# TuringLang/NormalizingFlows.jl

Measured on AMD Instinct MI355X. Metric: elbo_samples_per_sec, higher is better.
Workload: dtype f32; 1 GPU; reverse-KL ELBO step: RealNVP d=64, 8 affine couplings, conditioner 32-64-64-32 (hdims [64,64]), diag-Gaussian target, Philox base draws, Adam; batch_per_gpu=65536, global_batch=65536, params=133632, parallelism=dp1 (sample-sharded, one all-reduce of P+1 floats per step), nf_comm_size=1, lib_comm_hung=False, step_form=nf_elbo_step (whole iteration inside the library), init=Glorot-uniform weights, zero biases (Flux default), weight_cache=nf_ctx_set_weight_cache(ctx, 1), as train_flow's loop sets it

## Files before the change

normalizingflows.jl_amd/csrc/nf_api.hip:

```cpp
#include <cmath>
#include <cstdlib>

#include "nf_common.h"

int nf_launch_base_sample(nf_ctx *, int, int, long, uint64_t, uint64_t, uint32_t, void *, void *);
int nf_launch_base_logpdf(nf_ctx *, int, int, long, const void *, void *);
int nf_launch_base_unwhiten(nf_ctx *, int dtype, int kind, int d, long N, const void *mu, const void *scale, void *x);
int nf_launch_base_general_logpdf(nf_ctx *, int dtype, int kind, int d, long N, const void *mu, const void *scale, double logdet,
                                  const void *x, void *logq_out, void *corr_out, void *zbuf);
int nf_launch_base_general_score(nf_ctx *, int dtype, int kind, int d, long N, const void *mu, const void *scale, double logdet,
                                 const void *x, void *logq_out, void *score_out, double gscale, void *zbuf);
long nf_target_nblocks(long N);
int nf_launch_target(nf_ctx *, int, const nf_target *, int, long, const void *, const void *, const void *, void *,
                     void *, double, void *, double *, double, int joint_d);
long nf_sum2_nblocks(long N);
int nf_launch_sum2(nf_ctx *, int, long, const void *, const void *, void *, double *, double);
int nf_launch_finish_sum(nf_ctx *, const double *, long, int, double *, float *, double *, unsigned *bump = nullptr);
int nf_launch_reduce_slabs(nf_ctx *, int, const void *, int, long, void *);
long nf_adam_nblocks(long P);
int nf_launch_adam(nf_ctx *, int, void *, const void *, void *, void *, long, double, double, double, double, long,
                   double *);
int nf_launch_sgd(nf_ctx *, int, void *, const void *, void *, long, double, double, double *);
int nf_launch_fill(nf_ctx *, int, void *, long, double);
int nf_launch_base_sample_tiled(nf_ctx *, int d, long N, uint64_t seed, uint64_t off, uint32_t stream, float *xt, float *logq);
// ... 12 lines not shown
long nf_affine_chain_grid(nf_ctx *, long N);
int nf_affine_chain_elbo(nf_ctx *, const nf_flow_desc *, long N, uint64_t seed, uint64_t off, uint32_t stream,
                         const nf_target *target, float *yt, float *gt, double gscale, double *partial,
                         double pscale, float *stash = nullptr, const uint32_t *stream_ptr = nullptr);
long nf_affine_epilogue_blocks(const nf_flow_desc *desc);
bool nf_affine_chain_fkl_ok(const nf_flow_desc *desc);
int nf_affine_chain_fkl(nf_ctx *, const nf_flow_desc *, const float *ys, long N, float *gt, double gscale, double *partial,
                        double pscale, float *stash);
int nf_affine_epilogue(nf_ctx *, const nf_flow_desc *, int mode, const float *slab, int nslab, float *g, const double *lpart,
                       int nlpart, float *theta, float *m, float *v, double lr, double b1, double b2, double eps, unsigned t_val,
                       unsigned *t_ptr, double *gpart);
size_t nf_affine_stash_floats(const nf_flow_desc *desc, long N);
bool nf_affine_stash_pays(const nf_flow_desc *desc);
bool nf_affine_fused_ok(const nf_flow_desc *desc);
int nf_affine_bwd_stashed(nf_ctx *, const nf_flow_desc *, float *stash, float *ybar, const float *lbar, float lbar_const, long N,
                          float *slab, long slab_stride, int grid, bool inv_dir = false);
long nf_affine_slab_floats(const nf_flow_desc *desc);
int nf_affine_reduce_slabs(nf_ctx *, const nf_flow_desc *, const float *slab, int nslab, float *g,
                           const double *lpart = nullptr, int nlpart = 0, float *lout = nullptr);
int nf_affine_bwd(nf_ctx *, const nf_flow_desc *, int k, const float *theta, float *y, float *ybar, const float *lbar,
                  float lbar_const, long N, float *slab, long slab_stride, int grid);
int nf_affine_bwd_all(nf_ctx *, const nf_flow_desc *, float *y, float *ybar, const float *lbar, float lbar_const, long N,
                      float *slab, long slab_stride, int grid, bool inv_dir = false);

bool nf_wide_supported(const nf_flow_desc *desc);
int nf_wide_pack(nf_ctx *, const nf_flow_desc *, const float *theta);
int nf_wide_apply(nf_ctx *, const nf_flow_desc *, int k, bool inverse, float *xt, long N, float *ladj, int accumulate);
size_t nf_wide_bwd_ws_floats(nf_ctx *, const nf_flow_desc *, long N);
int nf_wide_bwd(nf_ctx *, const nf_flow_desc *, float *state, float *gbar, const float *lbar, float lbar_const, long N,
                float *ws, float *g_out, bool inv_dir = false);
size_t nf_wide_train_ws_floats(nf_ctx *, const nf_flow_desc *, long N);
// ... 1068 lines not shown

  if (tiled) {
    float *zt = (float *)z, *gt = (float *)gbar;
    NF_TRY(nf_launch_layout_convert(ctx, desc->d, N, (const float *)ys, zt, 1));
    if (stash) {
      NF_TRY(coupling_pack(ctx, desc, (const float *)theta));
      const long stride = coupling_slab_floats(ctx, desc, N);
      long nslab = 0, npart = 0;
      for (long o = 0; o < N; o += stash_nc) {
        const long nc = N - o < stash_nc ? N - o : stash_nc;
        const int gc = coupling_bwd_grid(ctx, desc, nc);
        NF_TRY(nf_affine_chain(ctx, desc, true, zt + o * desc->d, nc, (float *)ladj + o, stash));
        NF_TRY(nf_launch_target_tiled(ctx, &q0, desc->d, nc, zt + o * desc->d, nullptr, (const float *)ladj + o, gt + o * desc->d, -inv,
                                      nullptr, partial + npart, -inv));
        NF_TRY(nf_affine_bwd_stashed(ctx, desc, stash, gt + o * desc->d, nullptr, (float)(-inv), nc, (float *)slab + nslab * stride,
                                     stride, gc, true));
        nslab += gc;
        npart += nf_target_tiled_nblocks(nc);
      }
      NF_TRY(nf_launch_finish_sum(ctx, partial, npart, 0, nullptr, (float *)out + P, nullptr));
      return nf_affine_reduce_slabs(ctx, desc, (const float *)slab, (int)nslab, (float *)out);
    }
    NF_TRY(coupling_chain_tiled(ctx, desc, true, (const float *)theta, zt, N, (float *)ladj, -1, rqs_tape));
    NF_TRY(nf_launch_target_tiled(ctx, &q0, desc->d, N, zt, nullptr, (const float *)ladj, gt, -inv, nullptr, partial, -inv));
    NF_TRY(nf_launch_finish_sum(ctx, partial, nb, 0, nullptr, (float *)out + P, nullptr));
    return coupling_inv_bwd(ctx, desc, (const float *)theta, zt, gt, (float)(-inv), N, (float *)slab, grid, (float *)out, rqs_tape);
  }
  if (hf) {
    NF_TRY(nf_hf_apply(ctx, desc, 0, nf_layer_count(desc), true, theta, ys, N, z, ladj));
    NF_TRY(nf_launch_target(ctx, dt, &q0, desc->d, N, z, nullptr, ladj, nullptr, gbar, -inv, nullptr, partial, -inv, 0));
    NF_TRY(nf_hf_bwd_inv(ctx, desc, theta, ys, gbar, -inv, N, out, fws));
// ... 458 lines not shown
  (void)result;
  char *slab = cv.take<char>(slabf * es);
  char *sws = cv.take<char>(simple_ws);
  float *stash = stash_b ? cv.take<float>(stash_b / 4) : nullptr;
  void *rqs_tape = rqs_b ? (void *)cv.take<char>(rqs_b) : nullptr;

  if (fusable) {
    float *xt = (float *)x, *gt = (float *)gbar;
    NF_TRY(coupling_pack(ctx, desc, (const float *)theta));
    if (stash) {
      const long stride = coupling_slab_floats(ctx, desc, N);
      long nslab = 0, npart = 0;
      for (long o = 0; o < N; o += stash_nc) {
        const long nc = N - o < stash_nc ? N - o : stash_nc;
        const int gc = coupling_bwd_grid(ctx, desc, nc);
        NF_TRY(fused_chain_elbo(ctx, desc, target, nc, seed, sample_offset + (uint64_t)o, stream_id, xt + o * desc->d,
                                gt + o * desc->d, -inv, partial + npart, -inv, stash));
        NF_TRY(nf_affine_bwd_stashed(ctx, desc, stash, gt + o * desc->d, nullptr, (float)(-inv), nc,
                                     (float *)slab + nslab * stride, stride, gc));
        nslab += gc;
        npart += nf_affine_chain_grid(ctx, nc);
      }
      return nf_affine_reduce_slabs(ctx, desc, (const float *)slab, (int)nslab, (float *)out, partial, (int)npart, (float *)out + P);
    }
    NF_TRY(fused_chain_elbo(ctx, desc, target, N, seed, sample_offset, stream_id, xt, gt, -inv, partial, -inv,
                            is_nsf(desc) ? (float *)rqs_tape : nullptr));
    if (is_nsf(desc)) {
      NF_TRY(nf_launch_finish_sum(ctx, partial, fused_chain_grid(ctx, desc, N), 0, nullptr, (float *)out + P, nullptr));
      return realnvp_bwd(ctx, desc, (const float *)theta, xt, gt, nullptr, (float)(-inv), N, (float *)slab, grid, (float *)out,
                         nullptr, 0, nullptr, rqs_tape);
    }
    return realnvp_bwd(ctx, desc, (const float *)theta, xt, gt, nullptr, (float)(-inv), N, (float *)slab, grid, (float *)out,
                       partial, (int)nf_affine_chain_grid(ctx, N), (float *)out + P);
  }
// ... 19 lines not shown
      NF_TRY(nf_launch_base_logpdf_tiled(ctx, desc->d, N, xt, (float *)logq));
    } else {
      NF_TRY(nf_launch_base_sample_tiled(ctx, desc->d, N, seed, sample_offset, stream_id, xt, (float *)logq));
    }
    if (stash) {
      NF_TRY(coupling_pack(ctx, desc, (const float *)theta));
      const long stride = coupling_slab_floats(ctx, desc, N);
      long nslab = 0, npart = 0;
      for (long o = 0; o < N; o += stash_nc) {
        const long nc = N - o < stash_nc ? N - o : stash_nc;
        const int gc = coupling_bwd_grid(ctx, desc, nc);
        NF_TRY(nf_affine_chain(ctx, desc, false, xt + o * desc->d, nc, (float *)ladj + o, stash));
        NF_TRY(nf_launch_target_tiled(ctx, target, desc->d, nc, xt + o * desc->d, (const float *)logq + o, (const float *)ladj + o,
                                      gt + o * desc->d, -inv, nullptr, partial + npart, -inv));
        NF_TRY(nf_affine_bwd_stashed(ctx, desc, stash, gt + o * desc->d, nullptr, (float)(-inv), nc,
                                     (float *)slab + nslab * stride, stride, gc));
        nslab += gc;
        npart += nf_target_tiled_nblocks(nc);
      }
      NF_TRY(nf_launch_finish_sum(ctx, partial, npart, 0, nullptr, (float *)out + P, nullptr));
      return nf_affine_reduce_slabs(ctx, desc, (const float *)slab, (int)nslab, (float *)out);
    }
    NF_TRY(coupling_chain_tiled(ctx, desc, false, (const float *)theta, xt, N, (float *)ladj, -1, rqs_tape));
    NF_TRY(nf_launch_target_tiled(ctx, target, desc->d, N, xt, (const float *)logq, (const float *)ladj, gt, -inv,
                                  nullptr, partial, -inv));
    NF_TRY(nf_launch_finish_sum(ctx, partial, nb, 0, nullptr, (float *)out + P, nullptr));
    NF_TRY(realnvp_bwd(ctx, desc, (const float *)theta, xt, gt, nullptr, (float)(-inv), N, (float *)slab, grid,
                       (float *)out, nullptr, 0, nullptr, rqs_tape));
  } else {
    if (simple_step) {
      NF_TRY(nf_target_check(target, desc->d));
// ... 83 lines not shown
  for (int i = 0; i < d->n_hidden && i < 4; ++i) mix((unsigned long long)d->hdims[i]);
  return h | (1ull << 63);
}
static bool step_fusable(nf_ctx *ctx, const nf_flow_desc *desc, const nf_target *target, long N) {
  constexpr bool off = false;
  if (off || flow_base(desc) || is_composite(desc) || desc->dtype != NF_DTYPE_F32) return false;
  if (!(desc->kind == NF_KIND_REALNVP && nf_affine_supported(desc))) return false;
  if (!elbo_fusable(desc, target, nullptr)) return false;
  return affine_stash_chunk(ctx, desc, N) > 0;
}
static size_t step_fused_need(nf_ctx *ctx, const nf_flow_desc *desc, long N) {
  const size_t te = tiled_elems(desc, N);
  const long nb = nf_target_tiled_nblocks(N);
  const long nb_alloc = nb < ctx->num_cu ? ctx->num_cu : nb;
  const long snc = affine_stash_chunk(ctx, desc, N);
  return 2 * carve_bytes(te * 4) + carve_bytes((size_t)nb_alloc * 8) +
         carve_bytes(chunked_slab_floats(ctx, desc, N, snc, coupling_slab_floats(ctx, desc, N)) * 4) +
         carve_bytes(snc ? affine_stash_bytes(ctx, desc, snc) : 0) + carve_bytes((size_t)nf_affine_epilogue_blocks(desc) * 8);
}
static int elbo_step_fused(nf_ctx *ctx, const nf_flow_desc *desc, const nf_target *target, float *theta, float *m, float *v,
                           long N, uint64_t seed, uint32_t step_val, uint32_t *step_ptr, double lr, double beta1, double beta2,
                           double eps) {
  const long P = nf_param_count(desc);
  const int world = ctx->comm ? ctx->comm_size : 1;
  const long Ng = N * world;
  const uint64_t off0 = (uint64_t)(ctx->comm ? ctx->comm_rank : 0) * (uint64_t)N;
  const double inv = 1.0 / (double)Ng;
  const size_t te = tiled_elems(desc, N);
  const long nb = nf_target_tiled_nblocks(N);
  const long nb_alloc = nb < ctx->num_cu ? ctx->num_cu : nb;
  const long stash_nc = affine_stash_chunk(ctx, desc, N);
  const long stride = coupling_slab_floats(ctx, desc, N);
  const size_t slabf = chunked_slab_floats(ctx, desc, N, stash_nc, stride);
  const size_t stash_b = affine_stash_bytes(ctx, desc, stash_nc);
  const long eblocks = nf_affine_epilogue_blocks(desc);
  NF_TRY(nf_ws_reserve(ctx, step_fused_need(ctx, desc, N)));
  Carver cv(ctx->ws);
  float *xt = cv.take<float>(te);
  float *gt = cv.take<float>(te);
  double *partial = cv.take<double>(nb_alloc);
  float *slab = cv.take<float>(slabf);
  float *stash = cv.take<float>(stash_b / 4);
  double *gpart = cv.take<double>(eblocks);
  float *gbuf = (float *)ctx->gbuf;
  constexpr bool repack = false;
  if (repack || !ctx->wimg_cache ||
      !(ctx->wimg && ctx->wimg_owner == (const void *)theta && ctx->wimg_sig == flow_sig(desc))) {
    NF_TRY(coupling_pack(ctx, desc, theta));
  }
  long nslab = 0, npart = 0;
  for (long o = 0; o < N; o += stash_nc) {
    const long nc = N - o < stash_nc ? N - o : stash_nc;
    const int gc = coupling_bwd_grid(ctx, desc, nc);
    NF_TRY(nf_affine_chain_elbo(ctx, desc, nc, seed, off0 + (uint64_t)o, step_val, target,
                                xt + o * desc->d, gt + o * desc->d, -inv, partial + npart, -inv, stash, step_ptr));
    NF_TRY(nf_affine_bwd_stashed(ctx, desc, stash, gt + o * desc->d, nullptr, (float)(-inv), nc, slab + nslab * stride, stride, gc));
    nslab += gc;
    npart += nf_affine_chain_grid(ctx, nc);
  }
  if (world == 1) {
    NF_TRY(nf_affine_epilogue(ctx, desc, 3, slab, (int)nslab, gbuf, partial, (int)npart, theta, m, v, lr, beta1, beta2, eps, step_val,
                              step_ptr, gpart));
  } else {
    NF_TRY(nf_affine_epilogue(ctx, desc, 1, slab, (int)nslab, gbuf, partial, (int)npart, nullptr, nullptr, nullptr, lr, beta1, beta2,
                              eps, step_val, nullptr, gpart));
    NF_TRY(nf_allreduce_grad_loss(ctx, NF_DTYPE_F32, gbuf, P + 1));
    NF_TRY(nf_affine_epilogue(ctx, desc, 2, nullptr, 0, gbuf, nullptr, 0, theta, m, v, lr, beta1, beta2, eps, step_val, step_ptr,
                              gpart));
  }
  NF_TRY(nf_launch_finish_sum(ctx, gpart, eblocks, 1, nullptr, gbuf + P + 1, nullptr, step_ptr));
  ctx->wimg_owner = theta;
// ... 230 lines not shown
  NF_TRY(nf_ws_reserve(ctx, fkl_step_need(ctx, desc, N)));
  Carver cv(ctx->ws);
  float *gt = cv.take<float>(tiled_elems(desc, N));
  double *partial = cv.take<double>(fkl_step_npart(ctx, N, stash_nc));
  float *slab = cv.take<float>(chunked_slab_floats(ctx, desc, N, stash_nc, stride));
  float *stash = cv.take<float>(affine_stash_bytes(ctx, desc, stash_nc) / 4);
  double *gpart = cv.take<double>(eblocks);
  float *gbuf = (float *)ctx->gbuf;
  if (!ctx->wimg_cache || !(ctx->wimg && ctx->wimg_owner == (const void *)theta && ctx->wimg_sig == flow_sig(desc)))
    NF_TRY(coupling_pack(ctx, desc, theta));
  long nslab = 0, npart = 0;
  for (long o = 0; o < N; o += stash_nc) {
    const long nc = N - o < stash_nc ? N - o : stash_nc;
    const int gc = coupling_bwd_grid(ctx, desc, nc);
    NF_TRY(nf_affine_chain_fkl(ctx, desc, ys + o * desc->d, nc, gt + o * desc->d, -inv, partial + npart, -inv, stash));
    NF_TRY(nf_affine_bwd_stashed(ctx, desc, stash, gt + o * desc->d, nullptr, (float)(-inv), nc, slab + nslab * stride, stride, gc, true));
    nslab += gc;
    npart += nf_affine_chain_grid(ctx, nc);
  }
  if (world == 1) {
    NF_TRY(nf_affine_epilogue(ctx, desc, 3, slab, (int)nslab, gbuf, partial, (int)npart, theta, m, v, lr, beta1, beta2, eps, step_val,
                              step_ptr, gpart));
  } else {
    NF_TRY(nf_affine_epilogue(ctx, desc, 1, slab, (int)nslab, gbuf, partial, (int)npart, nullptr, nullptr, nullptr, lr, beta1, beta2,
                              eps, step_val, nullptr, gpart));
    NF_TRY(nf_allreduce_grad_loss(ctx, NF_DTYPE_F32, gbuf, P + 1));
    NF_TRY(nf_affine_epilogue(ctx, desc, 2, nullptr, 0, gbuf, nullptr, 0, theta, m, v, lr, beta1, beta2, eps, step_val, step_ptr,
                              gpart));
  }
  NF_TRY(nf_launch_finish_sum(ctx, gpart, eblocks, 1, nullptr, gbuf + P + 1, nullptr, step_ptr));
  ctx->wimg_owner = theta;
// ... 225 lines not shown
```

normalizingflows.jl_amd/csrc/nf_coupling.hip:

```cpp
#include <cmath>
#include <cstdlib>

#include "nf_common.h"
#ifdef NF_COUPLING_SPLIT_SCALAR
#define NF_SPLIT_SCALAR
#endif
#ifdef NF_COUPLING_SLOPE_SCALAR
#define NF_SLOPE_SCALAR
#endif
#include "nf_mfma.h"
#include "nf_pack.h"
#include "nf_philox.h"
#include "nf_target_epilogue.h"

int nf_target_check(const nf_target *t, int d);

struct CouplingArgs {
  const float *theta;
  const float *img_s, *img_t;
  long long *trace;
  NetDims s, t;
  int d, c, m, par_t;
  long N;
};
// ... 532 lines not shown
          NF_CH_STAMP(tr, 4);
          buf ^= 1;
          continue;
        } else if (INVERSE ? (half == 1) : (half == 0)) {
          (void)x1_is_O;
          ls = coupling_step<G, INVERSE>(img_s, img_t, O, E, l31, hi);
        } else {
          ls = coupling_step<G, INVERSE>(img_s, img_t, E, O, l31, hi);
        }
        lsum += ls;
        __syncthreads();
        buf ^= 1;
      }
    }
    if (live) {
      if constexpr (!FKL) {
#pragma unroll
        for (int b = 0; b < G::CB; ++b)
#pragma unroll
          for (int r = 0; r < 16; ++r) {
            tile_store(io, tile_soff(b, r, 0), E[b][r]);
            tile_store(io, tile_soff(b, r, 1), O[b][r]);
          }
      }
      lsum += __shfl_xor(lsum, 32);
      if (!FUSED) {
        if (hi == 0 && valid) ladj[j] = INVERSE ? -lsum : lsum;
      }
    }
    if constexpr (FKL) {
      const TileIO gio = make_tile_io(fa.gt, tl, a.d, l31, hi);
// ... 491 lines not shown

template <class G, bool FULL>
__global__ __launch_bounds__(256, 1) void k_affine_bwd(CouplingArgs a, float *__restrict__ y, float *__restrict__ ybar,
                                                       const float *__restrict__ lbar, float lbar_const,
                                                       float *__restrict__ slab, long slab_stride) {
  extern __shared__ __attribute__((aligned(16))) float lds[];
  bwd_coupling<G, FULL>(a, y, ybar, lbar, lbar_const, slab, slab_stride, lds);
}

struct BwdAllArgs {
  const float *wimg;
  const unsigned char *wimg_b6t;
  long long *trace;
  int d, ncoup;
  long N;
};
template <class G, bool FULL, bool INVD>
__global__ __launch_bounds__(256, 1) void k_affine_bwd_all(BwdAllArgs aa, float *__restrict__ y, float *__restrict__ ybar,
                                                           const float *__restrict__ lbar, float lbar_const,
                                                           float *__restrict__ slab, long slab_stride) {
  extern __shared__ __attribute__((aligned(16))) float lds[];
#pragma unroll 1
  for (int step = 0; step < aa.ncoup; ++step) {
    const int k = INVD ? aa.ncoup - 1 - step : step;
    CouplingArgs a;
    a.theta = nullptr;
    a.img_s = aa.wimg + (size_t)(2 * k) * G::SIZE;
    a.img_t = a.img_s + G::SIZE;
    a.trace = k == 0 ? aa.trace : nullptr;
    a.d = aa.d;
// ... 417 lines not shown
#define NF_PAIR_BUF D6_BUF
#define NF_PAIR_PUT(NB, buf, s) split_to_lds<NB>(buf, s, l31, hi)
#define NF_PAIR_DW(IB, OB, as, buf, w, b) dw_accumulate_t6<IB, OB>(as, buf, w, b, l31, hi)
#endif
template <class G, bool PB6 = false, bool DW6 = false>
struct BwdPairLds {
  static_assert(!DW6 || (PB6 && G::CB <= 2 && G::H1B <= 2 && G::H2B <= 2), "triple buffers hold two blocks");
  static constexpr int D3 = 0, D2 = D3 + G::CB * 32 * NF_TS, D1 = D2 + G::H2B * 32 * NF_TS;
  static constexpr int PAIR = DW6 ? 2 * NF_PAIR_BUF / 4 : D1 + G::H1B * 32 * NF_TS;
  static constexpr int PAIRS = 4;
  static constexpr int IMG = PB6 ? B6TGeo<G>::BYTES / 4 : G::SIZE;
  static constexpr int FLOATS = (IMG + PAIRS * PAIR) > PAIRS * G::SIZE ? (IMG + PAIRS * PAIR) : PAIRS * G::SIZE;
  static constexpr size_t BYTES = (size_t)FLOATS * sizeof(float);
};

template <class G, bool PHASE_S, bool FULL, bool INVD, bool SLIM, bool PB6 = false, bool DW6 = false>
__device__ __forceinline__ void pair_produce(const CouplingArgs &a, const float *__restrict__ img, float *__restrict__ sp,
                                             StashFirst<G> &f, float *stash, int k, int ncoup, float *__restrict__ ybar,
                                             const float *__restrict__ lbar, float lbar_const, long tile, long next_tile,
                                             bool live, int l31, int hi, int par, long long *tr = nullptr) {
  using SG = StashGeo<G, SLIM>;
  using L = BwdPairLds<G, PB6, DW6>;
  char *bufa = reinterpret_cast<char *>(sp) + par * NF_PAIR_BUF, *bufb = reinterpret_cast<char *>(sp) + (par ^ 1) * NF_PAIR_BUF;
  if (!live) {
    __syncthreads();
    __syncthreads();
    __syncthreads();
    return;
  }
  NF_TS_STAMP(0);
  const long j = tile * NF_TILE + l31;
  const bool valid = FULL ? true : j < a.N;
  const int par_c = 1 - a.par_t;
  const TileIO gio = make_tile_io(ybar, tile, a.d, l31, hi);
  const StashIO st = make_stash_io(stash, tile * ncoup + k, SG::SIZE, true, l31, hi);
  constexpr int nbase = SG::NET0 + (PHASE_S ? 0 : SG::NETSZ);
  f32x16 g1[G::CB];
#pragma unroll
  for (int b = 0; b < G::CB; ++b)
#pragma unroll
    for (int r = 0; r < 16; ++r) g1[b][r] = tile_load(gio, tile_soff(b, r, a.par_t));
  const u32x4 mk = __builtin_amdgcn_raw_buffer_load_b128(st.rs, (hi * 32 + l31) * 16, (nbase + SG::MSK) * 4, 0);
  f32x16 gold[G::MB];
#pragma unroll
  for (int b = 0; b < G::MB; ++b)
#pragma unroll
    for (int r = 0; r < 16; ++r) gold[b][r] = tile_load(gio, tile_soff(b, r, par_c));
  const float lb = valid ? (lbar ? lbar[FULL ? j : (j < a.N ? j : 0)] : lbar_const) : 0.f;
  f32x16 d3[G::CB];
#pragma unroll
  for (int b = 0; b < G::CB; ++b)
#pragma unroll
    for (int r = 0; r < 16; ++r) {
      const bool ok = (b * 32 + nf_row(r, hi) < a.c) && valid;
      const float gv = g1[b][r];
      if (!PHASE_S) {
        d3[b][r] = ok ? (INVD ? -gv : gv) : 0.f;
      } else if (INVD) {
        const float sv = f.sv[b][r];
        tile_store(gio, tile_soff(b, r, a.par_t), nf_fdiv(gv, nf_exp(sv)));
        d3[b][r] = ok ? -(gv * f.uv[b][r] + lb) * (1.f - sv * sv) : 0.f;
      } else {
        const float sv = f.sv[b][r];
        tile_store(gio, tile_soff(b, r, a.par_t), gv * nf_exp(sv));
        d3[b][r] = ok ? (gv * f.uv[b][r] + lb) * (1.f - sv * sv) : 0.f;
      }
    }
  SplitC<DW6 ? G::CB : 1> s3;
  if constexpr (DW6) {
    split_C<G::CB>(d3, s3);
    NF_PAIR_PUT(G::CB, bufa, s3);
  } else {
    tile_to_scratch<G::CB>(sp + L::D3, d3, l31, hi);
  }
  unsigned m1[G::H1B], m2[G::H2B];
#pragma unroll
  for (int b = 0; b < G::H1B; ++b) m1[b] = mk[b];
#pragma unroll
  for (int b = 0; b < G::H2B; ++b) m2[b] = mk[2 + b];
  NF_TS_STAMP(1);
  __syncthreads();
  NF_TS_STAMP(2);
// ... 51 lines not shown
  if constexpr (DW6) dense_bwd_x_b6s<G::H1B, G::H2B>(wt + B6TGeo<G>::T2, s2, d1, l31, hi);
  else if constexpr (PB6) dense_bwd_x_b6<G::H1B, G::H2B>(wt + B6TGeo<G>::T2, d2, d1, l31, hi);
  else dense_bwd_x<G::H1B, G::H2B>(img + G::W2, d2, d1, l31, hi);
  apply_lrelu_grad<G::H1B>(d1, m1);
  if constexpr (DW6) {
    split_C<G::H1B>(d1, s1);
    NF_PAIR_PUT(G::H1B, bufa, s1);
  } else {
    tile_to_scratch<G::H1B>(sp + L::D1, d1, l31, hi);
  }
  }
  NF_TS_STAMP(5);
  __syncthreads();
  NF_TS_STAMP(6);
  if (PHASE_S && next_tile >= 0) stash_issue_first<G, SLIM>(f, stash, k, ncoup, next_tile, l31, hi);
  f32x16 g2[G::MB];
  if constexpr (DW6) dense_bwd_x_b6s<G::MB, G::H1B>(wt + B6TGeo<G>::T1, s1, g2, l31, hi);
  else if constexpr (PB6) dense_bwd_x_b6<G::MB, G::H1B>(wt + B6TGeo<G>::T1, d1, g2, l31, hi);
  else dense_bwd_x<G::MB, G::H1B>(img + G::W1, d1, g2, l31, hi);
#pragma unroll
  for (int b = 0; b < G::MB; ++b)
#pragma unroll
    for (int r = 0; r < 16; ++r) tile_store(gio, tile_soff(b, r, par_c), gold[b][r] + g2[b][r]);
  NF_TS_STAMP(7);
}

template <int NA, int NB>
__device__ __forceinline__ void consumer_split_and_request(const StashIO &st, int base, int voff, const float (&at)[NA][16], SplitT<NA> &s,
                                                           float (&bt)[NB][16]) {
  constexpr int NS = 2 * NA, NL = 4 * NB;
#pragma unroll
  for (int i = 0; i < NS; ++i) {
    const int ib = i >> 1, g = i & 1;
    float v[8];
#pragma unroll
    for (int j = 0; j < 8; ++j) v[j] = at[ib][8 * g + j];
#pragma unroll
    for (int l = i * NL / NS; l < (i + 1) * NL / NS; ++l) {
// ... 250 lines not shown
    if constexpr (PB6)
      stage_packed<BT::BYTES / 4, 512>(img, reinterpret_cast<const float *>(aa.wimg_b6t + (size_t)(2 * k + (is_s ? 0 : 1)) * BT::BYTES), tid);
    else
      stage_packed<G::SIZE, 512>(img, aa.wimg + (size_t)(2 * k + (is_s ? 0 : 1)) * G::SIZE, tid);
  };
  const long ntiles = (aa.N + NF_TILE - 1) / NF_TILE;
  const long tile0 = (long)blockIdx.x * 4 + pair, tstride = (long)gridDim.x * 4;
  const long wg0 = (long)blockIdx.x * 4;
  const int rounds = wg0 < ntiles ? (int)((ntiles - wg0 + tstride - 1) / tstride) : 0;
  if (role == 0) {
    StashFirst<G> f;
    if (INVD && tile0 < ntiles) stash_issue_first<G, SLIM>(f, stash, aa.ncoup - 1, aa.ncoup, tile0, l31, hi);
#pragma unroll 1
    for (int step = 0; step < aa.ncoup; ++step) {
      const int k = INVD ? aa.ncoup - 1 - step : step;
      CouplingArgs a;
      a.theta = nullptr;
      a.img_s = aa.wimg + (size_t)(2 * k) * G::SIZE;
      a.img_t = a.img_s + G::SIZE;
      a.trace = nullptr;
      a.d = aa.d;
      a.par_t = k & 1;
      a.c = (k & 1) ? aa.d / 2 : (aa.d + 1) / 2;
      a.m = aa.d - a.c;
      a.N = aa.N;
#pragma unroll 1
      for (int phase = 0; phase < 2; ++phase) {
        const bool is_s = INVD ? phase == 0 : phase == 1;
#ifdef NF_KERNEL_TRACE
        long long *trb = (aa.trace && blockIdx.x == 0 && tid == 64 * NF_TRACE_PAIR && step == 0) ? aa.trace + 32 + phase * 8 : nullptr;
#endif
        NF_TSB(0);
        stage_image(k, is_s);
        NF_TSB(1);
        __syncthreads();
        NF_TSB(2);
#pragma unroll 1
        for (int it = 0; it < rounds; ++it) {
          const long tile = tile0 + (long)it * tstride;
          const long nt = tile + tstride < ntiles ? tile + tstride : -1;
#ifdef NF_KERNEL_TRACE
          long long *tr = (aa.trace && blockIdx.x == 0 && tid == 64 * NF_TRACE_PAIR && step == 0 && it < 2) ? aa.trace + phase * 16 + it * 8 : nullptr;
#else
          long long *tr = nullptr;
#endif
          if (!is_s) pair_produce<G, false, FULL, INVD, SLIM, PB6, DW6>(a, img, sp, f, stash, k, aa.ncoup, ybar, lbar, lbar_const, tile, nt, tile < ntiles, l31, hi, it & 1, tr);
          else pair_produce<G, true, FULL, INVD, SLIM, PB6, DW6>(a, img, sp, f, stash, k, aa.ncoup, ybar, lbar, lbar_const, tile, nt, tile < ntiles, l31, hi, it & 1, tr);
        }
        NF_TSB(3);
        __syncthreads();
        NF_TSB(4);
        if (tile0 < ntiles) {
          if (!INVD && !is_s) stash_issue_first<G, SLIM>(f, stash, k, aa.ncoup, tile0, l31, hi);
          if (INVD && !is_s && step + 1 < aa.ncoup) stash_issue_first<G, SLIM>(f, stash, k - 1, aa.ncoup, tile0, l31, hi);
        }
        __syncthreads();
        NF_TSB(5);
        pair_slab_write<G>(lds, slab + (long)k * 2 * G::SIZE + ((long)blockIdx.x * slab_stride + (is_s ? 0 : 1) * (long)G::SIZE), tid);
        NF_TSB(6);
        __syncthreads();
        NF_TSB(7);
      }
    }
// ... 356 lines not shown
  }
  return (int)hipGetLastError();
}

long nf_affine_chain_grid(nf_ctx *ctx, long N) {
  const long ngroups = ((N + NF_TILE - 1) / NF_TILE + 7) / 8;
  long grid = ngroups < ctx->num_cu ? ngroups : ctx->num_cu;
  return grid < 1 ? 1 : grid;
}

int nf_affine_chain_elbo(nf_ctx *ctx, const nf_flow_desc *desc, long N, uint64_t seed, uint64_t off, uint32_t stream,
                         const nf_target *target, float *yt, float *gt, double gscale, double *partial,
                         double pscale, float *stash, const uint32_t *stream_ptr) {
  const int size = geo_size(desc);
  if (!size || !ctx->wimg) return NF_ERR_UNSUPPORTED;
  NF_TRY(nf_target_check(target, desc->d));
  const float *mu = (const float *)target->p0, *var = (const float *)target->p1;
  FusedArgs fa;
  fa.tkind = target->kind; fa.ts0 = (float)target->s0; fa.ts1 = (float)target->s1;
  fa.stash = stash;
  fa.trace = (long long *)ctx->trace;
  fa.stream_ptr = stream_ptr;
  fa.k0 = (uint32_t)seed; fa.k1 = (uint32_t)(seed >> 32); fa.stream = stream; fa.off = off;
  fa.mu = mu; fa.var = var; fa.gt = gt; fa.gscale = (float)gscale; fa.partial = partial; fa.pscale = pscale;
  const bool b6 = fwd_b6(stash != nullptr);
  if (size == NetGeo<1, 1, 1, 1>::SIZE)
    return b6 ? launch_chain<NetGeo<1, 1, 1, 1>, false, true>(ctx, desc, false, yt, N, nullptr, &fa)
              : launch_chain<NetGeo<1, 1, 1, 1>>(ctx, desc, false, yt, N, nullptr, &fa);
  if (stash && stash_slim(size))
    return b6 ? launch_chain<NetGeo<1, 2, 2, 1>, true, true>(ctx, desc, false, yt, N, nullptr, &fa)
// ... 96 lines not shown
  return (int)hipGetLastError();
}

int nf_affine_bwd_all(nf_ctx *ctx, const nf_flow_desc *desc, float *y, float *ybar, const float *lbar, float lbar_const,
                      long N, float *slab, long slab_stride, int grid, bool inv_dir) {
  if (nf_deep_geo_id(desc)) return nf_deep_bwd(ctx, desc, 0, 2 * desc->nlayers, y, ybar, lbar, lbar_const, N, slab, slab_stride, grid, inv_dir);
  const int size = geo_size(desc);
  if (!size || !ctx->wimg || desc->n_hidden != 2) return NF_ERR_UNSUPPORTED;
  BwdAllArgs aa;
  aa.wimg = (const float *)ctx->wimg;
  aa.wimg_b6t = nullptr;
  aa.trace = (long long *)ctx->trace;
  aa.d = desc->d;
  aa.ncoup = 2 * desc->nlayers;
  aa.N = N;
  const bool h64 = size != NetGeo<1, 1, 1, 1>::SIZE;
  const bool full = desc->d == 64 && N % NF_TILE == 0;
  if (inv_dir) {
    if (h64)
      return full ? launch_bwd_all_v<NetGeo<1, 2, 2, 1>, true, true>(ctx, aa, y, ybar, lbar, lbar_const, slab, slab_stride, grid)
                  : launch_bwd_all_v<NetGeo<1, 2, 2, 1>, false, true>(ctx, aa, y, ybar, lbar, lbar_const, slab, slab_stride, grid);
    return launch_bwd_all_v<NetGeo<1, 1, 1, 1>, false, true>(ctx, aa, y, ybar, lbar, lbar_const, slab, slab_stride, grid);
  }
  if (h64)
    return full ? launch_bwd_all_v<NetGeo<1, 2, 2, 1>, true>(ctx, aa, y, ybar, lbar, lbar_const, slab, slab_stride, grid)
                : launch_bwd_all_v<NetGeo<1, 2, 2, 1>, false>(ctx, aa, y, ybar, lbar, lbar_const, slab, slab_stride, grid);
  return full ? launch_bwd_all_v<NetGeo<1, 1, 1, 1>, true>(ctx, aa, y, ybar, lbar, lbar_const, slab, slab_stride, grid)
              : launch_bwd_all_v<NetGeo<1, 1, 1, 1>, false>(ctx, aa, y, ybar, lbar, lbar_const, slab, slab_stride, grid);
}

// ... 50 lines not shown
                     lbar_const, slab, slab_stride);
  return (int)hipGetLastError();
}
template <class G, bool FULL, bool INVD>
static int launch_bwd_pair(nf_ctx *ctx, const nf_flow_desc *desc, const BwdAllArgs &aa, float *stash, float *ybar, const float *lbar,
                           float lbar_const, float *slab, long slab_stride, int grid) {
  static const bool fp32 = std::getenv("NF_BWD_FP32") != nullptr;
  if (stash_slim(G::SIZE)) return launch_bwd_pair_v<G, FULL, INVD, true, false>(ctx, desc, aa, stash, ybar, lbar, lbar_const, slab, slab_stride, grid);
  static const bool dw_fp32 = std::getenv("NF_BWD_DW_FP32") != nullptr;
  if (fp32) return launch_bwd_pair_v<G, FULL, INVD, false, false>(ctx, desc, aa, stash, ybar, lbar, lbar_const, slab, slab_stride, grid);
  return dw_fp32 ? launch_bwd_pair_v<G, FULL, INVD, false, true>(ctx, desc, aa, stash, ybar, lbar, lbar_const, slab, slab_stride, grid)
                 : launch_bwd_pair_v<G, FULL, INVD, false, true, true>(ctx, desc, aa, stash, ybar, lbar, lbar_const, slab, slab_stride, grid);
}

int nf_affine_bwd_stashed(nf_ctx *ctx, const nf_flow_desc *desc, float *stash, float *ybar, const float *lbar, float lbar_const,
                          long N, float *slab, long slab_stride, int grid, bool inv_dir) {
  const int size = geo_size(desc);
  if (!size || !ctx->wimg || desc->n_hidden != 2 || !stash) return NF_ERR_UNSUPPORTED;
  BwdAllArgs aa;
  aa.wimg = (const float *)ctx->wimg;
  aa.wimg_b6t = nullptr;
  aa.trace = (long long *)ctx->trace;
  aa.d = desc->d;
  aa.ncoup = 2 * desc->nlayers;
  aa.N = N;
  const bool h64 = size != NetGeo<1, 1, 1, 1>::SIZE;
  const bool full = desc->d == 64 && N % NF_TILE == 0;
  static const bool no_pair = std::getenv("NF_BWD_NO_PAIR") != nullptr;
  if (h64 && !no_pair) {
    using GP = NetGeo<1, 2, 2, 1>;
    if (inv_dir)
      return full ? launch_bwd_pair<GP, true, true>(ctx, desc, aa, stash, ybar, lbar, lbar_const, slab, slab_stride, grid)
                  : launch_bwd_pair<GP, false, true>(ctx, desc, aa, stash, ybar, lbar, lbar_const, slab, slab_stride, grid);
    return full ? launch_bwd_pair<GP, true, false>(ctx, desc, aa, stash, ybar, lbar, lbar_const, slab, slab_stride, grid)
                : launch_bwd_pair<GP, false, false>(ctx, desc, aa, stash, ybar, lbar, lbar_const, slab, slab_stride, grid);
  }
  if (inv_dir) {
    if (h64)
      return full ? launch_bwd_stashed_v<NetGeo<1, 2, 2, 1>, true, true>(ctx, aa, stash, ybar, lbar, lbar_const, slab, slab_stride, grid, desc)
                  : launch_bwd_stashed_v<NetGeo<1, 2, 2, 1>, false, true>(ctx, aa, stash, ybar, lbar, lbar_const, slab, slab_stride, grid, desc);
// ... 19 lines not shown
```

Before: 117.7 million samples/s.

## Skip unused output writes and park gradient tiles in registers across pair rounds

When the stashed forward path is used, the fused chain no longer writes the transformed samples (xt), and the workspace buffer for them is dropped. The stashed backward kernel gets a no_xbar flag so the last coupling skips writing the input cotangent, which is never consumed. In the forward-direction pair kernel, the first two tile rounds keep g1 and g2 gradient tiles in registers between the S and T phases instead of round-tripping them through global memory. This cuts global-memory traffic at the cost of higher register pressure and more template instantiations.

Result: faster. 119.9 million samples/s (median of 6 runs) (+1.9%).

```diff
diff --git a/normalizingflows.jl_amd/csrc/nf_api.hip b/normalizingflows.jl_amd/csrc/nf_api.hip
--- a/normalizingflows.jl_amd/csrc/nf_api.hip
+++ b/normalizingflows.jl_amd/csrc/nf_api.hip
@@ -50,7 +50,7 @@
 bool nf_affine_stash_pays(const nf_flow_desc *desc);
 bool nf_affine_fused_ok(const nf_flow_desc *desc);
 int nf_affine_bwd_stashed(nf_ctx *, const nf_flow_desc *, float *stash, float *ybar, const float *lbar, float lbar_const, long N,
-                          float *slab, long slab_stride, int grid, bool inv_dir = false);
+                          float *slab, long slab_stride, int grid, bool inv_dir = false, bool no_xbar = false);
 long nf_affine_slab_floats(const nf_flow_desc *desc);
 int nf_affine_reduce_slabs(nf_ctx *, const nf_flow_desc *, const float *slab, int nslab, float *g,
                            const double *lpart = nullptr, int nlpart = 0, float *lout = nullptr);
@@ -1149,7 +1149,7 @@
         NF_TRY(nf_launch_target_tiled(ctx, &q0, desc->d, nc, zt + o * desc->d, nullptr, (const float *)ladj + o, gt + o * desc->d, -inv,
                                       nullptr, partial + npart, -inv));
         NF_TRY(nf_affine_bwd_stashed(ctx, desc, stash, gt + o * desc->d, nullptr, (float)(-inv), nc, (float *)slab + nslab * stride,
-                                     stride, gc, true));
+                                     stride, gc, true, true));
         nslab += gc;
         npart += nf_target_tiled_nblocks(nc);
       }
@@ -1638,10 +1638,10 @@
       for (long o = 0; o < N; o += stash_nc) {
         const long nc = N - o < stash_nc ? N - o : stash_nc;
         const int gc = coupling_bwd_grid(ctx, desc, nc);
-        NF_TRY(fused_chain_elbo(ctx, desc, target, nc, seed, sample_offset + (uint64_t)o, stream_id, xt + o * desc->d,
+        NF_TRY(fused_chain_elbo(ctx, desc, target, nc, seed, sample_offset + (uint64_t)o, stream_id, nullptr,
                                 gt + o * desc->d, -inv, partial + npart, -inv, stash));
         NF_TRY(nf_affine_bwd_stashed(ctx, desc, stash, gt + o * desc->d, nullptr, (float)(-inv), nc,
-                                     (float *)slab + nslab * stride, stride, gc));
+                                     (float *)slab + nslab * stride, stride, gc, false, true));
         nslab += gc;
         npart += nf_affine_chain_grid(ctx, nc);
       }
@@ -1691,7 +1691,7 @@
         NF_TRY(nf_launch_target_tiled(ctx, target, desc->d, nc, xt + o * desc->d, (const float *)logq + o, (const float *)ladj + o,
                                       gt + o * desc->d, -inv, nullptr, partial + npart, -inv));
         NF_TRY(nf_affine_bwd_stashed(ctx, desc, stash, gt + o * desc->d, nullptr, (float)(-inv), nc,
-                                     (float *)slab + nslab * stride, stride, gc));
+                                     (float *)slab + nslab * stride, stride, gc, false, true));
         nslab += gc;
         npart += nf_target_tiled_nblocks(nc);
       }
@@ -1805,7 +1805,7 @@
   const long nb = nf_target_tiled_nblocks(N);
   const long nb_alloc = nb < ctx->num_cu ? ctx->num_cu : nb;
   const long snc = affine_stash_chunk(ctx, desc, N);
-  return 2 * carve_bytes(te * 4) + carve_bytes((size_t)nb_alloc * 8) +
+  return carve_bytes(te * 4) + carve_bytes((size_t)nb_alloc * 8) +
          carve_bytes(chunked_slab_floats(ctx, desc, N, snc, coupling_slab_floats(ctx, desc, N)) * 4) +
          carve_bytes(snc ? affine_stash_bytes(ctx, desc, snc) : 0) + carve_bytes((size_t)nf_affine_epilogue_blocks(desc) * 8);
 }
@@ -1827,7 +1827,6 @@
   const long eblocks = nf_affine_epilogue_blocks(desc);
   NF_TRY(nf_ws_reserve(ctx, step_fused_need(ctx, desc, N)));
   Carver cv(ctx->ws);
-  float *xt = cv.take<float>(te);
   float *gt = cv.take<float>(te);
   double *partial = cv.take<double>(nb_alloc);
   float *slab = cv.take<float>(slabf);
@@ -1844,8 +1843,9 @@
     const long nc = N - o < stash_nc ? N - o : stash_nc;
     const int gc = coupling_bwd_grid(ctx, desc, nc);
     NF_TRY(nf_affine_chain_elbo(ctx, desc, nc, seed, off0 + (uint64_t)o, step_val, target,
-                                xt + o * desc->d, gt + o * desc->d, -inv, partial + npart, -inv, stash, step_ptr));
-    NF_TRY(nf_affine_bwd_stashed(ctx, desc, stash, gt + o * desc->d, nullptr, (float)(-inv), nc, slab + nslab * stride, stride, gc));
+                                nullptr, gt + o * desc->d, -inv, partial + npart, -inv, stash, step_ptr));
+    NF_TRY(nf_affine_bwd_stashed(ctx, desc, stash, gt + o * desc->d, nullptr, (float)(-inv), nc, slab + nslab * stride, stride, gc,
+                                 false, true));
     nslab += gc;
     npart += nf_affine_chain_grid(ctx, nc);
   }
@@ -2106,7 +2106,8 @@
     const long nc = N - o < stash_nc ? N - o : stash_nc;
     const int gc = coupling_bwd_grid(ctx, desc, nc);
     NF_TRY(nf_affine_chain_fkl(ctx, desc, ys + o * desc->d, nc, gt + o * desc->d, -inv, partial + npart, -inv, stash));
-    NF_TRY(nf_affine_bwd_stashed(ctx, desc, stash, gt + o * desc->d, nullptr, (float)(-inv), nc, slab + nslab * stride, stride, gc, true));
+    NF_TRY(nf_affine_bwd_stashed(ctx, desc, stash, gt + o * desc->d, nullptr, (float)(-inv), nc, slab + nslab * stride, stride, gc, true,
+                                 true));
     nslab += gc;
     npart += nf_affine_chain_grid(ctx, nc);
   }
diff --git a/normalizingflows.jl_amd/csrc/nf_coupling.hip b/normalizingflows.jl_amd/csrc/nf_coupling.hip
--- a/normalizingflows.jl_amd/csrc/nf_coupling.hip
+++ b/normalizingflows.jl_amd/csrc/nf_coupling.hip
@@ -1,5 +1,6 @@
 #include <cmath>
 #include <cstdlib>
+#include <type_traits>
 
 #include "nf_common.h"
 #ifdef NF_COUPLING_SPLIT_SCALAR
@@ -570,7 +571,7 @@
       }
     }
     if (live) {
-      if constexpr (!FKL) {
+      if (!FKL && (!(FUSED && STASH) || xt != nullptr)) {
 #pragma unroll
         for (int b = 0; b < G::CB; ++b)
 #pragma unroll
@@ -1092,6 +1093,7 @@
   long long *trace;
   int d, ncoup;
   long N;
+  int no_xbar;
 };
 template <class G, bool FULL, bool INVD>
 __global__ __launch_bounds__(256, 1) void k_affine_bwd_all(BwdAllArgs aa, float *__restrict__ y, float *__restrict__ ybar,
@@ -1539,11 +1541,18 @@
   static constexpr size_t BYTES = (size_t)FLOATS * sizeof(float);
 };
 
-template <class G, bool PHASE_S, bool FULL, bool INVD, bool SLIM, bool PB6 = false, bool DW6 = false>
+#define NF_PAIR_PARK 2
+#define NF_PAIR_PARK_G1 1
+template <class G>
+struct PairPark {
+  f32x16 g1[NF_PAIR_PARK_G1][G::CB], g2[NF_PAIR_PARK][G::MB];
+};
+
+template <class G, bool PHASE_S, bool FULL, bool INVD, bool SLIM, bool PB6, bool DW6, int SLOT>
 __device__ __forceinline__ void pair_produce(const CouplingArgs &a, const float *__restrict__ img, float *__restrict__ sp,
-                                             StashFirst<G> &f, float *stash, int k, int ncoup, float *__restrict__ ybar,
-                                             const float *__restrict__ lbar, float lbar_const, long tile, long next_tile,
-                                             bool live, int l31, int hi, int par, long long *tr = nullptr) {
+                                             StashFirst<G> &f, PairPark<G> &pk, bool last, float *stash, int k, int ncoup,
+                                             float *__restrict__ ybar, const float *__restrict__ lbar, float lbar_const, long tile,
+                                             long next_tile, bool live, int l31, int hi, int par, long long *tr = nullptr) {
   using SG = StashGeo<G, SLIM>;
   using L = BwdPairLds<G, PB6, DW6>;
   char *bufa = reinterpret_cast<char *>(sp) + par * NF_PAIR_BUF, *bufb = reinterpret_cast<char *>(sp) + (par ^ 1) * NF_PAIR_BUF;
@@ -1560,17 +1569,31 @@
   const TileIO gio = make_tile_io(ybar, tile, a.d, l31, hi);
   const StashIO st = make_stash_io(stash, tile * ncoup + k, SG::SIZE, true, l31, hi);
   constexpr int nbase = SG::NET0 + (PHASE_S ? 0 : SG::NETSZ);
+  static_assert(!INVD || SLOT < 0, "the inverse direction parks nothing");
+  constexpr bool FIRST = PHASE_S == INVD;
+  constexpr bool parked = SLOT >= 0, parked1 = SLOT >= 0 && SLOT < NF_PAIR_PARK_G1;
+  constexpr int S2 = SLOT < 0 ? 0 : SLOT, S1 = parked1 ? SLOT : 0;
   f32x16 g1[G::CB];
-#pragma unroll
-  for (int b = 0; b < G::CB; ++b)
-#pragma unroll
-    for (int r = 0; r < 16; ++r) g1[b][r] = tile_load(gio, tile_soff(b, r, a.par_t));
+  if constexpr (FIRST || !parked1) {
+#pragma unroll
+    for (int b = 0; b < G::CB; ++b)
+#pragma unroll
+      for (int r = 0; r < 16; ++r) g1[b][r] = tile_load(gio, tile_soff(b, r, a.par_t));
+  } else {
+#pragma unroll
+    for (int b = 0; b < G::CB; ++b) g1[b] = pk.g1[S1][b];
+  }
   const u32x4 mk = __builtin_amdgcn_raw_buffer_load_b128(st.rs, (hi * 32 + l31) * 16, (nbase + SG::MSK) * 4, 0);
   f32x16 gold[G::MB];
-#pragma unroll
-  for (int b = 0; b < G::MB; ++b)
-#pragma unroll
-    for (int r = 0; r < 16; ++r) gold[b][r] = tile_load(gio, tile_soff(b, r, par_c));
+  if constexpr (!parked) {
+#pragma unroll
+    for (int b = 0; b < G::MB; ++b)
+#pragma unroll
+      for (int r = 0; r < 16; ++r) gold[b][r] = tile_load(gio, tile_soff(b, r, par_c));
+  }
+  TileIO gx = gio;
+  if constexpr (PHASE_S && !INVD)
+    gx.rs = __builtin_amdgcn_make_buffer_rsrc(ybar + tile * a.d * NF_TILE, 0, last ? 0 : a.d * NF_TILE * 4, 0x00020000);
   const float lb = valid ? (lbar ? lbar[FULL ? j : (j < a.N ? j : 0)] : lbar_const) : 0.f;
   f32x16 d3[G::CB];
 #pragma unroll
@@ -1587,10 +1610,14 @@
         d3[b][r] = ok ? -(gv * f.uv[b][r] + lb) * (1.f - sv * sv) : 0.f;
       } else {
         const float sv = f.sv[b][r];
-        tile_store(gio, tile_soff(b, r, a.par_t), gv * nf_exp(sv));
+        tile_store(gx, tile_soff(b, r, a.par_t), gv * nf_exp(sv));
         d3[b][r] = ok ? (gv * f.uv[b][r] + lb) * (1.f - sv * sv) : 0.f;
       }
     }
+  if constexpr (FIRST && parked1) {
+#pragma unroll
+    for (int b = 0; b < G::CB; ++b) pk.g1[S1][b] = g1[b];
+  }
   SplitC<DW6 ? G::CB : 1> s3;
   if constexpr (DW6) {
     split_C<G::CB>(d3, s3);
@@ -1672,14 +1699,34 @@
   __syncthreads();
   NF_TS_STAMP(6);
   if (PHASE_S && next_tile >= 0) stash_issue_first<G, SLIM>(f, stash, k, ncoup, next_tile, l31, hi);
+  if (last) {
+    NF_TS_STAMP(7);
+    return;
+  }
+  if constexpr (!FIRST && parked) {
+#pragma unroll
+    for (int b = 0; b < G::MB; ++b)
+#pragma unroll
+      for (int r = 0; r < 16; ++r) gold[b][r] = tile_load(gio, tile_soff(b, r, par_c));
+  }
   f32x16 g2[G::MB];
   if constexpr (DW6) dense_bwd_x_b6s<G::MB, G::H1B>(wt + B6TGeo<G>::T1, s1, g2, l31, hi);
   else if constexpr (PB6) dense_bwd_x_b6<G::MB, G::H1B>(wt + B6TGeo<G>::T1, d1, g2, l31, hi);
   else dense_bwd_x<G::MB, G::H1B>(img + G::W1, d1, g2, l31, hi);
-#pragma unroll
-  for (int b = 0; b < G::MB; ++b)
-#pragma unroll
-    for (int r = 0; r < 16; ++r) tile_store(gio, tile_soff(b, r, par_c), gold[b][r] + g2[b][r]);
+  if constexpr (!parked) {
+#pragma unroll
+    for (int b = 0; b < G::MB; ++b)
+#pragma unroll
+      for (int r = 0; r < 16; ++r) tile_store(gio, tile_soff(b, r, par_c), gold[b][r] + g2[b][r]);
+  } else if constexpr (FIRST) {
+#pragma unroll
+    for (int b = 0; b < G::MB; ++b) pk.g2[S2][b] = g2[b];
+  } else {
+#pragma unroll
+    for (int b = 0; b < G::MB; ++b)
+#pragma unroll
+      for (int r = 0; r < 16; ++r) tile_store(gio, tile_soff(b, r, par_c), (gold[b][r] + pk.g2[S2][b][r]) + g2[b][r]);
+  }
   NF_TS_STAMP(7);
 }
 
@@ -1960,6 +2007,8 @@
 #pragma unroll 1
     for (int step = 0; step < aa.ncoup; ++step) {
       const int k = INVD ? aa.ncoup - 1 - step : step;
+      const bool last = aa.no_xbar != 0 && step + 1 == aa.ncoup;
+      PairPark<G> pk;
       CouplingArgs a;
       a.theta = nullptr;
       a.img_s = aa.wimg + (size_t)(2 * k) * G::SIZE;
@@ -1981,8 +2030,8 @@
         NF_TSB(1);
         __syncthreads();
         NF_TSB(2);
-#pragma unroll 1
-        for (int it = 0; it < rounds; ++it) {
+        auto produce = [&](int it, auto slot) {
+          constexpr int SLOT = decltype(slot)::value;
           const long tile = tile0 + (long)it * tstride;
           const long nt = tile + tstride < ntiles ? tile + tstride : -1;
 #ifdef NF_KERNEL_TRACE
@@ -1990,9 +2039,18 @@
 #else
           long long *tr = nullptr;
 #endif
-          if (!is_s) pair_produce<G, false, FULL, INVD, SLIM, PB6, DW6>(a, img, sp, f, stash, k, aa.ncoup, ybar, lbar, lbar_const, tile, nt, tile < ntiles, l31, hi, it & 1, tr);
-          else pair_produce<G, true, FULL, INVD, SLIM, PB6, DW6>(a, img, sp, f, stash, k, aa.ncoup, ybar, lbar, lbar_const, tile, nt, tile < ntiles, l31, hi, it & 1, tr);
+          if (!is_s) pair_produce<G, false, FULL, INVD, SLIM, PB6, DW6, SLOT>(a, img, sp, f, pk, last, stash, k, aa.ncoup, ybar, lbar, lbar_const, tile, nt, tile < ntiles, l31, hi, it & 1, tr);
+          else pair_produce<G, true, FULL, INVD, SLIM, PB6, DW6, SLOT>(a, img, sp, f, pk, last, stash, k, aa.ncoup, ybar, lbar, lbar_const, tile, nt, tile < ntiles, l31, hi, it & 1, tr);
+        };
+        int it0 = 0;
+        if constexpr (!INVD) {
+          static_assert(NF_PAIR_PARK == 2, "one call per slot");
+          if (rounds > 0) produce(0, std::integral_constant<int, 0>{});
+          if (rounds > 1) produce(1, std::integral_constant<int, 1>{});
+          it0 = NF_PAIR_PARK;
         }
+#pragma unroll 1
+        for (int it = it0; it < rounds; ++it) produce(it, std::integral_constant<int, -1>{});
         NF_TSB(3);
         __syncthreads();
         NF_TSB(4);
@@ -2379,6 +2437,7 @@
                          double pscale, float *stash, const uint32_t *stream_ptr) {
   const int size = geo_size(desc);
   if (!size || !ctx->wimg) return NF_ERR_UNSUPPORTED;
+  if (!yt && !stash) return NF_ERR_ARG;
   NF_TRY(nf_target_check(target, desc->d));
   const float *mu = (const float *)target->p0, *var = (const float *)target->p1;
   FusedArgs fa;
@@ -2505,6 +2564,7 @@
   aa.d = desc->d;
   aa.ncoup = 2 * desc->nlayers;
   aa.N = N;
+  aa.no_xbar = 0;
   const bool h64 = size != NetGeo<1, 1, 1, 1>::SIZE;
   const bool full = desc->d == 64 && N % NF_TILE == 0;
   if (inv_dir) {
@@ -2585,7 +2645,7 @@
 }
 
 int nf_affine_bwd_stashed(nf_ctx *ctx, const nf_flow_desc *desc, float *stash, float *ybar, const float *lbar, float lbar_const,
-                          long N, float *slab, long slab_stride, int grid, bool inv_dir) {
+                          long N, float *slab, long slab_stride, int grid, bool inv_dir, bool no_xbar) {
   const int size = geo_size(desc);
   if (!size || !ctx->wimg || desc->n_hidden != 2 || !stash) return NF_ERR_UNSUPPORTED;
   BwdAllArgs aa;
@@ -2595,6 +2655,7 @@
   aa.d = desc->d;
   aa.ncoup = 2 * desc->nlayers;
   aa.N = N;
+  aa.no_xbar = no_xbar ? 1 : 0;
   const bool h64 = size != NetGeo<1, 1, 1, 1>::SIZE;
   const bool full = desc->d == 64 && N % NF_TILE == 0;
   static const bool no_pair = std::getenv("NF_BWD_NO_PAIR") != nullptr;
```
